# prstrive/SuRF

Hardware: AMD Instinct MI355X
Metric: rays/sec (576x800, 5-view, 128 samp/ray render, whole job) (higher is better)
Workload: dtype f32 (operands split exactly into 3 bf16 pieces, fp32 accumulate)

## Files before the change

### surf_amd/csrc/blend_split.hip

```cpp
#include <math.h>
#include <string.h>

#include "blend_raw.h"
#include "common.h"

namespace {

using namespace blend_raw;

constexpr int TILE = 32;
#ifndef SURF_BLEND_WPB
#define SURF_BLEND_WPB 8
#endif
constexpr int WPB = SURF_BLEND_WPB;

enum { L_RD0, L_RD2, L_B0S, L_B0V, L_B2, L_V0, L_V2, L_W0, L_R0, L_R2, N_L };
constexpr int NKS[N_L] = {1, 1, 3, 2, 4, 2, 2, 2, 3, 1};
constexpr int NT[N_L] = {1, 1, 2, 2, 1, 1, 1, 1, 1, 1};
constexpr int blk_off(int l) { int o = 0; for (int i = 0; i < l; ++i) o += NKS[i] * NT[i]; return o; }
constexpr int N_BLK = blk_off(N_L);
enum { B_RD0, B_RD2, B_B0_T0, B_B0_T1, B_B2, B_V0, B_V2, B_W0, B_R0, B_R2, N_BIAS };
enum { D_VIS, D_VIS2, D_RGB4, N_DOT };
template <int BB> constexpr int bias_off() { return N_BLK * BB; }
template <int BB> constexpr int dot_off() { return bias_off<BB>() + N_BIAS * 128; }
template <int BB> constexpr int scal_off() { return dot_off<BB>() + N_DOT * 128; }
template <int BB> constexpr int image_bytes() { return scal_off<BB>() + 16; }

constexpr float LOG2E = 1.44269504088896341f, LN2 = 0.69314718055994531f;

typedef __bf16 bf16x8 __attribute__((ext_vector_type(8)));
typedef __bf16 bf16x2 __attribute__((ext_vector_type(2)));
typedef _Float16 f16x8 __attribute__((ext_vector_type(8)));
typedef _Float16 f16x2 __attribute__((ext_vector_type(2)));
typedef float f32x2 __attribute__((ext_vector_type(2)));
typedef uint32_t u32x4 __attribute__((ext_vector_type(4)));

template <int NP>
struct FragT { u32x4 p[NP]; };

#ifndef SURF_BLEND_MRES
#define SURF_BLEND_MRES 1
#endif

#ifndef SURF_BLEND_MRES_MASK
#define SURF_BLEND_MRES_MASK 0x3ff
#endif
struct BPolBf3 {
  static constexpr int NP = 3, ID = 1, BB = NP * 1024, LANE_BYTES = 16;
  static constexpr bool MRES = SURF_BLEND_MRES != 0;
  static constexpr bool mres_at(int site) { return MRES && ((SURF_BLEND_MRES_MASK >> site) & 1); }
#ifndef SURF_BLEND_REG_VIEWS_BF3
#define SURF_BLEND_REG_VIEWS_BF3 2
#endif
// ... 331 lines not shown
#endif
}

template <class P> constexpr int lds_bytes() { return image_bytes<P::BB>(); }

constexpr int SLOT_GROUPS = 5;
constexpr int slot_floats(int ns) { return ns * SLOT_GROUPS * 64 * 4; }
#ifndef SURF_BLEND_LDS_VIEWS
#define SURF_BLEND_LDS_VIEWS 2
#endif
constexpr int VIEW_BYTES = SLOT_GROUPS * 64 * 16;
template <class P> constexpr int lds_views() {
  const int n = (160 * 1024 - lds_bytes<P>()) / (WPB * VIEW_BYTES);
  return n < SURF_BLEND_LDS_VIEWS ? n : SURF_BLEND_LDS_VIEWS;
}
struct Stage {
  float* slot;
  char* lds_v;
  int n_lds;
};

struct ViewState {
  float floc[12];
  float rd[4];
  float rgb[3];
  float ex;
  float mk;
};
template <class PtrT>
__device__ __forceinline__ void slot_store_at(PtrT p, const ViewState& s, int stride = 64) {
  p[0 * stride] = f32x4{s.floc[0], s.floc[1], s.floc[2], s.floc[3]};
  p[1 * stride] = f32x4{s.floc[4], s.floc[5], s.floc[6], s.floc[7]};
  p[2 * stride] = f32x4{s.floc[8], s.floc[9], s.floc[10], s.floc[11]};
  p[3 * stride] = f32x4{s.rd[0], s.rd[1], s.rd[2], s.rd[3]};
  p[4 * stride] = f32x4{s.rgb[0], s.rgb[1], s.rgb[2], s.mk != 0.f ? s.ex : -s.ex};
}
template <class PtrT>
__device__ __forceinline__ void slot_load_at(PtrT p, ViewState& s, int stride = 64) {
  f32x4 x[5];
#pragma unroll
  for (int g = 0; g < 5; ++g) x[g] = p[g * stride];
#pragma unroll
  for (int g = 0; g < 3; ++g) {
    s.floc[4 * g + 0] = x[g][0]; s.floc[4 * g + 1] = x[g][1]; s.floc[4 * g + 2] = x[g][2]; s.floc[4 * g + 3] = x[g][3];
  }
  s.rd[0] = x[3][0]; s.rd[1] = x[3][1]; s.rd[2] = x[3][2]; s.rd[3] = x[3][3];
  s.rgb[0] = x[4][0]; s.rgb[1] = x[4][1]; s.rgb[2] = x[4][2];
  s.mk = x[4][3] > 0.f ? 1.f : 0.f;
  s.ex = fabsf(x[4][3]);
}
typedef __attribute__((address_space(3))) f32x4* lds_f32x4_ptr;
struct ViewRegs { f32x4 x[5]; };
template <int NRV> struct RegViews { ViewRegs v0, v1, v2; };
template <int NRV>
__device__ __forceinline__ void slot_store(const Stage& g, int v, int lane, const ViewState& s, RegViews<NRV>& keep) {
  if (v < g.n_lds) { slot_store_at((lds_f32x4_ptr)(g.lds_v + v * VIEW_BYTES), s); return; }
  if (NRV > 0 && v == g.n_lds) { slot_store_at(&keep.v0.x[0], s, 1); return; }
  if (NRV > 1 && v == g.n_lds + 1) { slot_store_at(&keep.v1.x[0], s, 1); return; }
  if (NRV > 2 && v == g.n_lds + 2) { slot_store_at(&keep.v2.x[0], s, 1); return; }
  slot_store_at(reinterpret_cast<f32x4*>(g.slot + (int64_t)(v * SLOT_GROUPS) * 256 + lane * 4), s);
}
template <int NRV>
__device__ __forceinline__ void slot_load(const Stage& g, int v, int lane, ViewState& s, const RegViews<NRV>& keep) {
  if (v < g.n_lds) { slot_load_at((lds_f32x4_ptr)(g.lds_v + v * VIEW_BYTES), s); return; }
  if (NRV > 0 && v == g.n_lds) { slot_load_at(&keep.v0.x[0], s, 1); return; }
  if (NRV > 1 && v == g.n_lds + 1) { slot_load_at(&keep.v1.x[0], s, 1); return; }
  if (NRV > 2 && v == g.n_lds + 2) { slot_load_at(&keep.v2.x[0], s, 1); return; }
  slot_load_at(reinterpret_cast<const f32x4*>(g.slot + (int64_t)(v * SLOT_GROUPS) * 256 + lane * 4), s);
}

struct Geo {
  const float* mapA;
  const float* mapB;
  const float* mapC;
  int HA, WA, HB, WB;
  float scA, scB, cWA, cHA, cWB, cHB, rWA, rHA, rWB, rHB;
  int h;
};
__device__ __forceinline__ Geo make_geo(const BlendArgs& a, int h) {
  Geo g;
  g.h = h;
  g.mapA = h ? a.feats[2] : a.feats[0];
  g.mapB = h ? a.feats[3] : a.feats[1];
  g.mapC = h ? a.feats[2] : a.imgs;
  g.HA = h ? a.hw[4] : a.hw[0]; g.WA = h ? a.hw[5] : a.hw[1];
  g.HB = h ? a.hw[6] : a.hw[2]; g.WB = h ? a.hw[7] : a.hw[3];
  g.scA = h ? 0.25f : 1.0f; g.scB = h ? 0.125f : 0.5f;
  g.cWA = (float)(g.WA - 1) / 2.0f; g.cHA = (float)(g.HA - 1) / 2.0f; g.cWB = (float)(g.WB - 1) / 2.0f; g.cHB = (float)(g.HB - 1) / 2.0f;
  g.rWA = 1.0f / g.cWA; g.rHA = 1.0f / g.cHA; g.rWB = 1.0f / g.cWB; g.rHB = 1.0f / g.cHB;
  return g;
}
struct Fetch {
  Tap4 qA, qB, qC;
  TapGeom gA, gB;
  bool ok;
};
__device__ __forceinline__ void pass1_issue(const BlendArgs& a, const Geo& geo, int cam, float px, float py, float pz, float ax, float ay,
                                        float az, ViewState& st, Fetch& q) {
  const int h = geo.h;
  const float* __restrict__ mapA = geo.mapA;
  const float* __restrict__ mapB = geo.mapB;
  const int HA = geo.HA, WA = geo.WA, HB = geo.HB, WB = geo.WB;
  const float scA = geo.scA, scB = geo.scB, cWA = geo.cWA, cHA = geo.cHA, cWB = geo.cWB, cHB = geo.cHB;
  const float rWA = geo.rWA, rHA = geo.rHA, rWB = geo.rWB, rHB = geo.rHB;
  Tap4& qA = q.qA; Tap4& qB = q.qB; Tap4& qC = q.qC;
  TapGeom& gA = q.gA; TapGeom& gB = q.gB;
  (void)h;
  float bx = a.cpos[cam][0] - px, by = a.cpos[cam][1] - py, bz = a.cpos[cam][2] - pz;
  {
    const float nn = sqrtf(bx * bx + by * by + bz * bz) + 1e-6f;
    bx /= nn; by /= nn; bz /= nn;
  }
  const float ddx = ax - bx, ddy = ay - by, ddz = az - bz;
#ifdef SURF_BX_EXACT_RD
  {
    const float dn = fmaxf(sqrtf(ddx * ddx + ddy * ddy + ddz * ddz), 1e-6f);
    st.rd[0] = ddx / dn; st.rd[1] = ddy / dn; st.rd[2] = ddz / dn;
  }
#else
  {
    const float inv = __builtin_amdgcn_rcpf(fmaxf(__builtin_amdgcn_sqrtf(ddx * ddx + ddy * ddy + ddz * ddz), 1e-6f));
    st.rd[0] = ddx * inv; st.rd[1] = ddy * inv; st.rd[2] = ddz * inv;
  }
#endif
  st.rd[3] = ax * bx + ay * by + az * bz;
  const float* M = a.w2c[cam];
  const float X = M[0] * px + M[1] * py + M[2] * pz + M[3];
  const float Y = M[4] * px + M[5] * py + M[6] * pz + M[7];
  const float Z = M[8] * px + M[9] * py + M[10] * pz + M[11];
  const float* K = a.K[cam];
  const float qx = K[0] * X + K[1] * Y + K[2] * Z;
  const float qy = K[3] * X + K[4] * Y + K[5] * Z;
  const float qz = K[6] * X + K[7] * Y + K[8] * Z;
  const float u0 = qx / qz, v0 = qy / qz;
  bool ok = qz > 0.f;
  {
    const float u = u0 * scA, vv = v0 * scA;
    ok = ok && (u >= 0.f) && (u < (float)WA) && (vv >= 0.f) && (vv < (float)HA);
    const float nx = div_const(u, cWA, rWA) - 1.0f, ny = div_const(vv, cHA, rHA) - 1.0f;
    const float gx = ((nx + 1.0f) * (float)WA - 1.0f) * 0.5f, gy = ((ny + 1.0f) * (float)HA - 1.0f) * 0.5f;
    gA = tap_geom(HA, WA, gx, gy);
    tap_issue(qA, mapA + (int64_t)cam * HA * WA * 4, gA);
    tap_issue(qC, geo.mapC + (int64_t)cam * HA * WA * 4, gA);
  }
  {
    const float u = u0 * scB, vv = v0 * scB;
    ok = ok && (u >= 0.f) && (u < (float)WB) && (vv >= 0.f) && (vv < (float)HB);
    const float nx = div_const(u, cWB, rWB) - 1.0f, ny = div_const(vv, cHB, rHB) - 1.0f;
    const float gx = ((nx + 1.0f) * (float)WB - 1.0f) * 0.5f, gy = ((ny + 1.0f) * (float)HB - 1.0f) * 0.5f;
    gB = tap_geom(HB, WB, gx, gy);
    tap_issue(qB, mapB + (int64_t)cam * HB * WB * 4, gB);
  }
  q.ok = ok;
}
template <class P>
__device__ __forceinline__ bool pass1_finish(const Ctx& c, const Geo& geo, float s_abs, ViewState& st, const Fetch& q) {
  typedef typename P::Frag Frag;
  const int h = geo.h;
  const Tap4& qA = q.qA; const Tap4& qB = q.qB; const Tap4& qC = q.qC;
  const TapGeom& gA = q.gA; const TapGeom& gB = q.gB;
  bool ok = q.ok;
  float d12[12];
  {
    const float bin[2] = {h ? st.rd[1] : st.rd[0], h ? st.rd[3] : st.rd[2]};
    Frag fb, f8;
    frags_from<P, 2, 1>(bin, &fb);
    f32x16 acc1 = bias_row<P>(c, B_RD0);
    mma_layer<P, L_RD0, 0, 1>(c, acc1, &fb);
    elu_make_frags<P, 8, 0>(c, acc1, &f8);
    f32x16 acc2 = bias_row<P>(c, B_RD2);
    mma_layer<P, L_RD2, 0, 1>(c, acc2, &f8);
    elu_rows<12>(acc2, d12);
  }
  const f32x4 tA = tap_finish(qA, gA), tB = tap_finish(qB, gB);
  f32x4 tC = tap_finish(qC, gA);
  if (h != 0) tC = f32x4{0.f, 0.f, 0.f, 0.f};
  ok = ok && (__shfl_xor((int)ok, 32) != 0);
  st.mk = ok ? 1.f : 0.f;
  st.rgb[0] = tC[0]; st.rgb[1] = tC[1]; st.rgb[2] = tC[2];
  float g[12];
  if (h == 0) {
    g[0] = tC[0]; g[1] = tC[1]; g[2] = tC[2];
    g[3] = tA[0]; g[4] = tA[1]; g[5] = tA[2]; g[6] = tA[3];
    g[7] = tB[0]; g[8] = tB[1]; g[9] = tB[2]; g[10] = tB[3];
  } else {
    g[0] = tA[0]; g[1] = tA[1]; g[2] = tA[2]; g[3] = tA[3];
    g[4] = tB[0]; g[5] = tB[1]; g[6] = tB[2]; g[7] = tB[3];
    g[8] = g[9] = g[10] = 0.f;
  }
#pragma unroll
  for (int r = 0; r < 11; ++r) st.floc[r] = g[r] + d12[r];
  st.floc[11] = 0.f;
  st.ex = expf(s_abs * (st.rd[3] - 1.0f));
  return ok;
}

template <class P>
__global__ __launch_bounds__(WPB * 64, WPB / 4) void blend_split_kernel(BlendArgs a) {
  typedef typename P::Frag Frag;
  __shared__ __attribute__((aligned(16))) char lds[lds_bytes<P>() + WPB * lds_views<P>() * VIEW_BYTES];
  static_assert(lds_bytes<P>() % 16 == 0 && lds_bytes<P>() + WPB * lds_views<P>() * VIEW_BYTES <= 160 * 1024, "LDS");
  for (int o = threadIdx.x * 16; o < lds_bytes<P>(); o += WPB * 64 * 16)
    *reinterpret_cast<u32x4*>(lds + o) = *reinterpret_cast<const u32x4*>(a.w + o);
  __syncthreads();

  Ctx c0;
  const int lane = threadIdx.x & 63;
  const int j = lane & 31, h = lane >> 5;
  c0.lds = lds;
  c0.lane16 = lane * 16;
  c0.h64 = h * 64;
  c0.I0 = ident_frag(lane, 0);
  c0.I1 = ident_frag(lane, 1);
  const int NS = a.nv - 1;
  const int64_t wave_id = (int64_t)blockIdx.x * WPB + (threadIdx.x >> 6);
  const int64_t n_waves = (int64_t)gridDim.x * WPB;
  const int64_t n_pts = a.n_dev ? (int64_t)*a.n_dev : a.n;
  const int64_t n_tiles = (n_pts + TILE - 1) / TILE;
  Stage slot;
  slot.slot = a.scratch + wave_id * slot_floats(NS);
  slot.lds_v = lds + lds_bytes<P>() + (threadIdx.x >> 6) * (lds_views<P>() * VIEW_BYTES) + lane * 16;
  slot.n_lds = lds_views<P>();
  const float* scal = reinterpret_cast<const float*>(lds + scal_off<P::BB>());
  const float s_abs = scal[0], b_vis = scal[1], b_vis2 = scal[2], b_rgb4 = scal[3];

  const Geo geo = make_geo(a, h);

#ifdef SURF_BLEND_TIMING
  unsigned long long tprev = __builtin_readcyclecounter(), tacc[8] = {0, 0, 0, 0, 0, 0, 0, 0};
  const unsigned long long t_begin = tprev, rt_begin = __builtin_amdgcn_s_memrealtime();
#endif
  for (int64_t tile = wave_id; tile < n_tiles; tile += n_waves) {
    SURF_BT(0);
    const int64_t slot_i = tile * TILE + j;
    const int64_t sc = slot_i < n_pts ? slot_i : n_pts - 1;
    const int64_t i = a.idx ? (int64_t)a.idx[sc] : sc;
    const bool active = (slot_i < n_pts) && (!a.mask || a.mask[i] != 0);
    if (__ballot(active) == 0ull) continue;
    const float px = a.pts[i * 3 + 0], py = a.pts[i * 3 + 1], pz = a.pts[i * 3 + 2];

    float ax = a.cpos[0][0] - px, ay = a.cpos[0][1] - py, az = a.cpos[0][2] - pz;
    {
      const float nn = sqrtf(ax * ax + ay * ay + az * az) + 1e-6f;
      ax /= nn; ay /= nn; az /= nn;
    }
    int nvalid = 0;
    float emin = INFINITY;
    RegViews<P::REG_VIEWS> keep;
#pragma unroll 1
    for (int v = 0; v < NS; ++v) {
      const Ctx c = opaque(c0);
      ViewState st;
      Fetch q;
      pass1_issue(a, geo, v + 1, px, py, pz, ax, ay, az, st, q);
      nvalid += pass1_finish<P>(c, geo, s_abs, st, q) ? 1 : 0;
      emin = fminf(emin, st.ex);
      slot_store(slot, v, lane, st, keep);
    }
    if (a.n_valid && active && h == 0) a.n_valid[i] = (uint8_t)nvalid;
    SURF_BT(1);

    float wsum = 0.f;
    float mv[24];
#pragma unroll
    for (int ch = 0; ch < 24; ++ch) mv[ch] = 0.f;
#pragma unroll 1
    for (int v = 0; v < NS; ++v) {
      ViewState st;
      slot_load(slot, v, lane, st, keep);
      const float w = (st.ex - emin) * st.mk;
      wsum += w;
#pragma unroll
      for (int ch = 0; ch < 12; ++ch) mv[ch] += st.floc[ch] * w;
    }
    const float winv = 1.0f / (wsum + 1e-8f);
#pragma unroll
    for (int ch = 0; ch < 12; ++ch) mv[ch] *= winv;
#pragma unroll 1
    for (int v = 0; v < NS; ++v) {
      ViewState st;
      slot_load(slot, v, lane, st, keep);
      const float w = (st.ex - emin) * st.mk * winv;
#pragma unroll
      for (int ch = 0; ch < 12; ++ch) { const float d = st.floc[ch] - mv[ch]; mv[12 + ch] += w * (d * d); }
    }
    SURF_BT(2);
    f32x16 G0a, G0b;
    {
      const Ctx c = opaque(c0);
      G0a = bias_row<P>(c, B_B0_T0);
      G0b = bias_row<P>(c, B_B0_T1);
      Frag fm[3];
      make_frags<P, 24, 3, 1>(c, mv, fm);
      mma_layer<P, L_B0S, 0, 3>(c, G0a, fm);
      mma_layer<P, L_B0S, 1, 3>(c, G0b, fm);
    }

    float Mx = -INFINITY, Zs = 0.f, o_r = 0.f, o_g = 0.f, o_b = 0.f;
    SURF_BT(3);
#pragma unroll 1
    for (int v = 0; v < NS; ++v) {
      const Ctx c = opaque(c0);
      ViewState st;
      slot_load(slot, v, lane, st, keep);
      const float wv = (st.ex - emin) * st.mk * winv;
      f32x16 a0 = G0a, a1 = G0b;
      {
        Frag fl[2];
        make_frags<P, 12, 2, 2>(c, st.floc, fl);
        mma_layer<P, L_B0V, 0, 2>(c, a0, fl);
        mma_layer<P, L_B0V, 1, 2>(c, a1, fl);
      }
      f32x16 ax2 = bias_row<P>(c, B_B2);
      {
        Frag hf[2];
        elu_make_frags<P, 16, 3>(c, a0, hf);
        mma_blk<P, L_B2, 0, 0>(c, ax2, hf[0]);
        mma_blk<P, L_B2, 1, 0>(c, ax2, hf[1]);
        SURF_PHASE();
        elu_make_frags<P, 16, 4>(c, a1, hf);
        mma_blk<P, L_B2, 2, 0>(c, ax2, hf[0]);
        mma_blk<P, L_B2, 3, 0>(c, ax2, hf[1]);
        SURF_PHASE();
      }
      float x[16];
      elu_rows<16>(ax2, x);
      SURF_BT(4);
      float vis;
      {
        f32x16 at;
#pragma unroll
        for (int r = 0; r < 16; ++r) at[r] = 0.f;
        {
          Frag xf[2];
          make_frags<P, 16, 2, 5>(c, x, xf);
          mma_layer<P, L_V0, 0, 2>(c, at, xf);
        }
        const f32x16 bt = bias_row<P>(c, B_V0);
        f32x16 ar = bias_row<P>(c, B_V2);
        float vraw = 0.f;
        {
          float t16[16];
#pragma unroll
          for (int r = 0; r < 16; ++r) t16[r] = elu_t(fmaf(at[r], wv, bt[r]));
          const f32x16 dvis = dot_row<P>(c, D_VIS);
#pragma unroll
          for (int r = 0; r < 16; ++r) vraw = fmaf(dvis[r], t16[r], vraw);
          Frag tf[2];
          make_frags<P, 16, 2, 6>(c, t16, tf);
          mma_layer<P, L_V2, 0, 2>(c, ar, tf);
        }
        vraw += __shfl_xor(vraw, 32);
        vis = sigm(elu_x(vraw + b_vis)) * st.mk;
#pragma unroll
        for (int r = 0; r < 16; ++r) x[r] += elu_t(ar[r]);
      }
      SURF_BT(5);
      Frag rf[3];
      make_frags<P, 16, 2, 7>(c, x, rf);
      float vis2;
      {
        f32x16 aw;
#pragma unroll
        for (int r = 0; r < 16; ++r) aw[r] = 0.f;
        mma_layer<P, L_W0, 0, 2>(c, aw, rf);
        const f32x16 bw = bias_row<P>(c, B_W0);
        const f32x16 dvis2 = dot_row<P>(c, D_VIS2);
        float v2 = 0.f;
#pragma unroll
        for (int r = 0; r < 16; ++r) v2 = fmaf(dvis2[r], elu_t(fmaf(aw[r], vis, bw[r])), v2);
        v2 += __shfl_xor(v2, 32);
        vis2 = sigm(v2 + b_vis2) * st.mk;
      }
      SURF_BT(6);
      float rr;
      {
        f32x16 a16 = bias_row<P>(c, B_R0);
        {
          const float extra[3] = {h ? st.rd[0] : vis2, h ? st.rd[2] : st.rd[1], h ? 0.f : st.rd[3]};
          make_frags<P, 3, 1, 8>(c, extra, rf + 2);
          mma_layer<P, L_R0, 0, 3>(c, a16, rf);
        }
        f32x16 a8 = bias_row<P>(c, B_R2);
        {
          Frag f8;
          elu_make_frags<P, 8, 9>(c, a16, &f8);
          mma_layer<P, L_R2, 0, 1>(c, a8, &f8);
        }
        const f32x16 drgb4 = dot_row<P>(c, D_RGB4);
        rr = 0.f;
#pragma unroll
        for (int r = 0; r < 4; ++r) rr = fmaf(drgb4[r], elu_t(a8[r]), rr);
        rr += __shfl_xor(rr, 32);
        rr += b_rgb4;
      }
      if (st.mk == 0.f) rr = -1e9f;
      const float Mn = fmaxf(Mx, rr);
      const float scl = expf(Mx - Mn);
      const float e = expf(rr - Mn);
      Zs = Zs * scl + e;
      o_r = o_r * scl + e * st.rgb[0];
      o_g = o_g * scl + e * st.rgb[1];
      o_b = o_b * scl + e * st.rgb[2];
      Mx = Mn;
      SURF_BT(7);
    }
    if (active && h == 0) {
      a.color[i * 3 + 0] = o_r / Zs;
      a.color[i * 3 + 1] = o_g / Zs;
      a.color[i * 3 + 2] = o_b / Zs;
    }
  }
#ifdef SURF_BLEND_TIMING
  if (threadIdx.x == 0)
    for (int k = 0; k < 8; ++k) atomicAdd(&g_bphase[k], tacc[k]);
  if (threadIdx.x == 0 && blockIdx.x < 256) {
    g_bwg[blockIdx.x][0] = rt_begin;
    g_bwg[blockIdx.x][1] = __builtin_amdgcn_s_memrealtime();
  }
  if (threadIdx.x == 0 && blockIdx.x == 0) {
    g_bphase[8] = __builtin_readcyclecounter() - t_begin;
    g_bphase[9] = __builtin_amdgcn_s_memrealtime() - rt_begin;
  }
#endif
}

int grid_blocks(int64_t n) {
  const int64_t tiles = (n + TILE - 1) / TILE;
  const int64_t blocks = (tiles + WPB - 1) / WPB;
  return (int)(blocks < 256 ? blocks : 256);
}

inline uint16_t bf16_rne(float f) {
  uint32_t u;
  memcpy(&u, &f, 4);
  if ((u & 0x7fffffffu) > 0x7f800000u) return (uint16_t)((u >> 16) | 0x40);
  u += 0x7fffu + ((u >> 16) & 1u);
  return (uint16_t)(u >> 16);
}
inline float bf16_to_f(uint16_t b) {
  uint32_t u = (uint32_t)b << 16;
  float f;
  memcpy(&f, &u, 4);
  return f;
}
inline uint16_t f16_bits(float v) {
  _Float16 hh = (_Float16)v;
  uint16_t b;
  memcpy(&b, &hh, 2);
  return b;
}
inline float f16_to_f(uint16_t b) {
  _Float16 hh;
  memcpy(&hh, &b, 2);
  return (float)hh;
}
template <class P> void split_host(float v, uint16_t* p);
template <> void split_host<BPolBf3>(float v, uint16_t* p) {
  p[0] = bf16_rne(v);
  float r = v - bf16_to_f(p[0]);
  p[1] = bf16_rne(r);
  r = r - bf16_to_f(p[1]);
  p[2] = bf16_rne(r);
}
template <> void split_host<BPolH2>(float v, uint16_t* p) {
  p[0] = f16_bits(v);
  p[1] = f16_bits(v - f16_to_f(p[0]));
}
template <class P> void put_weight(unsigned char* out, int blk, int lane, int i, float v) {
  uint16_t p[P::NP];
  split_host<P>(v, p);
  for (int pc = 0; pc < P::NP; ++pc) reinterpret_cast<uint16_t*>(out + (int64_t)blk * P::BB + pc * 1024 + lane * 16)[i] = p[pc];
}
template <> void put_weight<BPolF32>(unsigned char* out, int blk, int lane, int i, float v) {
  reinterpret_cast<float*>(out + (int64_t)blk * BPolF32::BB + lane * 32)[i] = v;
}

// ... 29 lines not shown
  float* dots = reinterpret_cast<float*>(out + dot_off<P::BB>());
  float* scal = reinterpret_cast<float*>(out + scal_off<P::BB>());
  auto nat_row = [](int lim) { return [lim](int t, int rho) { const int f = 32 * t + rho; return f < lim ? f : -1; }; };
  auto nat_col = [](int lim) { return [lim](int m, int h) { const int f = hk(m / 16, m % 16, h); return f < lim ? f : -1; }; };
  auto natf = [](int lim) { return [lim](int r, int h) { const int f = hk(0, r, h); return f < lim ? f : -1; }; };
  auto dir_row = [](int t, int rho) { const int hr = (rho >> 2) & 1, r = (rho & 3) | ((rho >> 3) << 2); return loc_ch(r, hr); };

  pack_layer<P>(out, L_RD0, raw + R_RD0_W, 4, nat_row(16), [](int m, int h) { return m < 2 ? 2 * m + h : -1; });
  pack_rows(bias + B_RD0 * 32, raw + R_RD0_B, natf(16), LOG2E);
  pack_layer<P>(out, L_RD2, raw + R_RD2_W, 16, dir_row, nat_col(16));
  pack_rows(bias + B_RD2 * 32, raw + R_RD2_B, [](int r, int h) { return loc_ch(r, h); }, LOG2E);
  pack_layer<P>(out, L_B0S, raw + R_B0_W, 57, nat_row(64), [](int m, int h) {
    const int grp = m / 12, s = m % 12;
    const int ch = (grp < 2 && s < 11) ? loc_ch(s, h) : -1;
    return ch >= 0 ? grp * DF + ch : -1;
  });
  pack_rows(bias + B_B0_T0 * 32, raw + R_B0_B, [](int r, int h) { return hk(0, r, h); }, LOG2E);
  pack_rows(bias + B_B0_T1 * 32, raw + R_B0_B, [](int r, int h) { return hk(1, r, h); }, LOG2E);
  pack_layer<P>(out, L_B0V, raw + R_B0_W, 57, nat_row(64), [](int m, int h) {
    const int ch = m < 11 ? loc_ch(m, h) : -1;
    return ch >= 0 ? 2 * DF + ch : -1;
  });
  pack_layer<P>(out, L_B2, raw + R_B2_W, 64, nat_row(32), nat_col(64));
  pack_rows(bias + B_B2 * 32, raw + R_B2_B, natf(32), LOG2E);
  pack_layer<P>(out, L_V0, raw + R_V0_W, 32, nat_row(32), nat_col(32));
  pack_rows(bias + B_V0 * 32, raw + R_V0_B, natf(32), LOG2E);
  pack_layer<P>(out, L_V2, raw + R_V2_W, 32, nat_row(32), nat_col(32));
  pack_rows(bias + B_V2 * 32, raw + R_V2_B, natf(32), LOG2E);
  pack_rows(dots + D_VIS * 32, raw + R_V2_W + 32 * 32, natf(32), 1.0f);
  pack_layer<P>(out, L_W0, raw + R_W0_W, 32, nat_row(32), nat_col(32));
  pack_rows(bias + B_W0 * 32, raw + R_W0_B, natf(32), LOG2E);
  pack_rows(dots + D_VIS2 * 32, raw + R_W2_W, natf(32), 1.0f);
  pack_layer<P>(out, L_R0, raw + R_R0_W, 37, nat_row(16), [](int m, int h) {
    if (m < 16) return hk(0, m, h);
    if (m == 16) return h ? 33 : 32;
    if (m == 17) return h ? 35 : 34;
    if (m == 18) return h ? -1 : 36;
    return -1;
  });
  pack_rows(bias + B_R0 * 32, raw + R_R0_B, natf(16), LOG2E);
  pack_layer<P>(out, L_R2, raw + R_R2_W, 16, nat_row(8), nat_col(16));
  pack_rows(bias + B_R2 * 32, raw + R_R2_B, natf(8), LOG2E);
  pack_rows(dots + D_RGB4 * 32, raw + R_R4_W, [](int r, int h) { return r < 4 ? 4 * h + r : -1; }, 1.0f);
  scal[0] = fabsf(raw[R_S]);
  scal[1] = raw[R_V2_B + 32];
  scal[2] = raw[R_W2_B];
  scal[3] = raw[R_R4_B];
  return 0;
}

template <class P>
int launch(const BlendArgs& a, hipStream_t st) {
  dim3 grid(grid_blocks(a.n)), block(WPB * 64);
  hipLaunchKernelGGL((blend_split_kernel<P>), grid, block, 0, st, a);
  return surf_check_launch();
}

}

#ifdef SURF_BLEND_TIMING
extern "C" int surf_debug_blend_wg(unsigned long long* out) {
  return hipMemcpyFromSymbol(out, HIP_SYMBOL(g_bwg), sizeof(unsigned long long) * 512) == hipSuccess ? 0 : 100;
}
extern "C" int surf_debug_blend_phases(unsigned long long* out, int reset) {
  if (hipMemcpyFromSymbol(out, HIP_SYMBOL(g_bphase), sizeof(unsigned long long) * 10) != hipSuccess) return 100;
  if (reset) {
    unsigned long long z[10] = {0, 0, 0, 0, 0, 0, 0, 0, 0, 0};
    if (hipMemcpyToSymbol(HIP_SYMBOL(g_bphase), z, sizeof(z)) != hipSuccess) return 100;
  }
  return 0;
}
#endif

extern "C" int64_t surf_blend_split_packed_bytes(int precision) {
  if (precision == BPolBf3::ID) return image_bytes<BPolBf3::BB>();
  if (precision == BPolH2::ID) return image_bytes<BPolH2::BB>();
  if (precision == BPolF32::ID) return image_bytes<BPolF32::BB>();
  return SURF_E_ARG;
}

extern "C" int surf_blend_pack_weights_split(const float* h_raw, unsigned char* h_packed, int precision) {
  if (precision == BPolBf3::ID) return pack_weights<BPolBf3>(h_raw, h_packed);
  if (precision == BPolH2::ID) return pack_weights<BPolH2>(h_raw, h_packed);
  if (precision == BPolF32::ID) return pack_weights<BPolF32>(h_raw, h_packed);
  return SURF_E_ARG;
}

extern "C" int64_t surf_blend_split_scratch_bytes(int64_t n_points, int nv) {
  if (n_points <= 0 || nv < 2 || nv > SURF_MAX_VIEWS) return 0;
  return (int64_t)grid_blocks(n_points) * WPB * slot_floats(nv - 1) * (int64_t)sizeof(float);
}

static int blend_split_impl(const float* pts, const uint8_t* mask, const int32_t* idx, int64_t n, const int32_t* d_n,
                            const float* const* h_feats, const int* h_hw, int n_level, const float* imgs, int nv,
                            const float* h_intrs, const float* h_w2c, const float* h_c2w, const void* blend_w,
                            int precision, float* color, uint8_t* n_valid, void* scratch, void* stream) {
  if (!pts || !h_feats || !h_hw || !imgs || !h_intrs || !h_w2c || !h_c2w || !blend_w || !color || !scratch) return SURF_E_ARG;
  if (n <= 0 || nv < 2) return SURF_E_ARG;
  if (n_level != 4 || nv > SURF_MAX_VIEWS) return SURF_E_LIMIT;
  if (precision != BPolBf3::ID && precision != BPolH2::ID && precision != BPolF32::ID) return SURF_E_ARG;
  BlendArgs a;
  a.pts = pts; a.mask = mask; a.idx = idx; a.n = n; a.n_dev = d_n; a.imgs = imgs; a.w = (const unsigned char*)blend_w; a.color = color;
  a.n_valid = n_valid;
  a.scratch = (float*)scratch;
  a.nv = nv;
  for (int l = 0; l < 4; ++l) {
    if (!h_feats[l]) return SURF_E_ARG;
// ... 35 lines not shown
```

Baseline: 3.010 million.

## Share per-view geometry across wave halves and split register-view paths statically

Each wave half now computes the camera geometry (ray direction, exp weight, projection) for a different view, and the results are exchanged with ds_bpermute, so two views cost one geometry computation per lane. The register-kept views are peeled out of the runtime-indexed loops into static calls, which removes the dynamic branch chain in slot load and store and may help keep those views in registers. The tap selection in pass1_finish becomes per-element selects instead of a divergent branch. The price is extra cross-lane permutes and somewhat more complex control flow.

```diff
diff --git a/surf_amd/csrc/blend_split.hip b/surf_amd/csrc/blend_split.hip
--- a/surf_amd/csrc/blend_split.hip
+++ b/surf_amd/csrc/blend_split.hip
@@ -436,13 +436,24 @@
 typedef __attribute__((address_space(3))) f32x4* lds_f32x4_ptr;
 struct ViewRegs { f32x4 x[5]; };
 template <int NRV> struct RegViews { ViewRegs v0, v1, v2; };
-template <int NRV>
-__device__ __forceinline__ void slot_store(const Stage& g, int v, int lane, const ViewState& s, RegViews<NRV>& keep) {
+__device__ __forceinline__ void slot_store_mem(const Stage& g, int v, int lane, const ViewState& s) {
   if (v < g.n_lds) { slot_store_at((lds_f32x4_ptr)(g.lds_v + v * VIEW_BYTES), s); return; }
-  if (NRV > 0 && v == g.n_lds) { slot_store_at(&keep.v0.x[0], s, 1); return; }
-  if (NRV > 1 && v == g.n_lds + 1) { slot_store_at(&keep.v1.x[0], s, 1); return; }
-  if (NRV > 2 && v == g.n_lds + 2) { slot_store_at(&keep.v2.x[0], s, 1); return; }
   slot_store_at(reinterpret_cast<f32x4*>(g.slot + (int64_t)(v * SLOT_GROUPS) * 256 + lane * 4), s);
+}
+__device__ __forceinline__ void slot_load_mem(const Stage& g, int v, int lane, ViewState& s) {
+  if (v < g.n_lds) { slot_load_at((lds_f32x4_ptr)(g.lds_v + v * VIEW_BYTES), s); return; }
+  slot_load_at(reinterpret_cast<const f32x4*>(g.slot + (int64_t)(v * SLOT_GROUPS) * 256 + lane * 4), s);
+}
+template <int NRV, class KeepT, class MemF, class RegF>
+__device__ __forceinline__ void for_views_in_order(int NS, int n_lds, KeepT& keep, MemF mem, RegF reg) {
+  const int n0 = NS < n_lds ? NS : n_lds;
+#pragma unroll 1
+  for (int v = 0; v < n0; ++v) mem(v);
+  if (NRV > 0 && NS > n_lds) reg(n_lds, keep.v0);
+  if (NRV > 1 && NS > n_lds + 1) reg(n_lds + 1, keep.v1);
+  if (NRV > 2 && NS > n_lds + 2) reg(n_lds + 2, keep.v2);
+#pragma unroll 1
+  for (int v = n_lds + NRV; v < NS; ++v) mem(v);
 }
 template <int NRV>
 __device__ __forceinline__ void slot_load(const Stage& g, int v, int lane, ViewState& s, const RegViews<NRV>& keep) {
@@ -479,8 +490,57 @@
   TapGeom gA, gB;
   bool ok;
 };
-__device__ __forceinline__ void pass1_issue(const BlendArgs& a, const Geo& geo, int cam, float px, float py, float pz, float ax, float ay,
-                                        float az, ViewState& st, Fetch& q) {
+struct P1Geom {
+  float rd[4];
+  float ex, u0, v0;
+  int front;
+};
+__device__ __forceinline__ P1Geom pass1_geom(const BlendArgs& a, int cam, float px, float py, float pz, float ax, float ay, float az,
+                                             float s_abs) {
+  P1Geom g;
+  float bx = a.cpos[cam][0] - px, by = a.cpos[cam][1] - py, bz = a.cpos[cam][2] - pz;
+  {
+    const float nn = sqrtf(bx * bx + by * by + bz * bz) + 1e-6f;
+    bx /= nn; by /= nn; bz /= nn;
+  }
+  const float ddx = ax - bx, ddy = ay - by, ddz = az - bz;
+#ifdef SURF_BX_EXACT_RD
+  {
+    const float dn = fmaxf(sqrtf(ddx * ddx + ddy * ddy + ddz * ddz), 1e-6f);
+    g.rd[0] = ddx / dn; g.rd[1] = ddy / dn; g.rd[2] = ddz / dn;
+  }
+#else
+  {
+    const float inv = __builtin_amdgcn_rcpf(fmaxf(__builtin_amdgcn_sqrtf(ddx * ddx + ddy * ddy + ddz * ddz), 1e-6f));
+    g.rd[0] = ddx * inv; g.rd[1] = ddy * inv; g.rd[2] = ddz * inv;
+  }
+#endif
+  g.rd[3] = ax * bx + ay * by + az * bz;
+  g.ex = expf(s_abs * (g.rd[3] - 1.0f));
+  const float* M = a.w2c[cam];
+  const float X = M[0] * px + M[1] * py + M[2] * pz + M[3];
+  const float Y = M[4] * px + M[5] * py + M[6] * pz + M[7];
+  const float Z = M[8] * px + M[9] * py + M[10] * pz + M[11];
+  const float* K = a.K[cam];
+  const float qx = K[0] * X + K[1] * Y + K[2] * Z;
+  const float qy = K[3] * X + K[4] * Y + K[5] * Z;
+  const float qz = K[6] * X + K[7] * Y + K[8] * Z;
+  g.u0 = qx / qz; g.v0 = qy / qz;
+  g.front = qz > 0.f ? 1 : 0;
+  return g;
+}
+__device__ __forceinline__ P1Geom geom_of_half(const P1Geom& g, int t, int lane) {
+  const int src = (((lane & 31) | (t << 5)) << 2);
+  P1Geom o;
+#pragma unroll
+  for (int k = 0; k < 4; ++k) o.rd[k] = __builtin_bit_cast(float, __builtin_amdgcn_ds_bpermute(src, __builtin_bit_cast(int, g.rd[k])));
+  o.ex = __builtin_bit_cast(float, __builtin_amdgcn_ds_bpermute(src, __builtin_bit_cast(int, g.ex)));
+  o.u0 = __builtin_bit_cast(float, __builtin_amdgcn_ds_bpermute(src, __builtin_bit_cast(int, g.u0)));
+  o.v0 = __builtin_bit_cast(float, __builtin_amdgcn_ds_bpermute(src, __builtin_bit_cast(int, g.v0)));
+  o.front = __builtin_amdgcn_ds_bpermute(src, g.front);
+  return o;
+}
+__device__ __forceinline__ void pass1_issue(const Geo& geo, int cam, const P1Geom& pg, ViewState& st, Fetch& q) {
   const int h = geo.h;
   const float* __restrict__ mapA = geo.mapA;
   const float* __restrict__ mapB = geo.mapB;
@@ -490,34 +550,10 @@
   Tap4& qA = q.qA; Tap4& qB = q.qB; Tap4& qC = q.qC;
   TapGeom& gA = q.gA; TapGeom& gB = q.gB;
   (void)h;
-  float bx = a.cpos[cam][0] - px, by = a.cpos[cam][1] - py, bz = a.cpos[cam][2] - pz;
-  {
-    const float nn = sqrtf(bx * bx + by * by + bz * bz) + 1e-6f;
-    bx /= nn; by /= nn; bz /= nn;
-  }
-  const float ddx = ax - bx, ddy = ay - by, ddz = az - bz;
-#ifdef SURF_BX_EXACT_RD
-  {
-    const float dn = fmaxf(sqrtf(ddx * ddx + ddy * ddy + ddz * ddz), 1e-6f);
-    st.rd[0] = ddx / dn; st.rd[1] = ddy / dn; st.rd[2] = ddz / dn;
-  }
-#else
-  {
-    const float inv = __builtin_amdgcn_rcpf(fmaxf(__builtin_amdgcn_sqrtf(ddx * ddx + ddy * ddy + ddz * ddz), 1e-6f));
-    st.rd[0] = ddx * inv; st.rd[1] = ddy * inv; st.rd[2] = ddz * inv;
-  }
-#endif
-  st.rd[3] = ax * bx + ay * by + az * bz;
-  const float* M = a.w2c[cam];
-  const float X = M[0] * px + M[1] * py + M[2] * pz + M[3];
-  const float Y = M[4] * px + M[5] * py + M[6] * pz + M[7];
-  const float Z = M[8] * px + M[9] * py + M[10] * pz + M[11];
-  const float* K = a.K[cam];
-  const float qx = K[0] * X + K[1] * Y + K[2] * Z;
-  const float qy = K[3] * X + K[4] * Y + K[5] * Z;
-  const float qz = K[6] * X + K[7] * Y + K[8] * Z;
-  const float u0 = qx / qz, v0 = qy / qz;
-  bool ok = qz > 0.f;
+  st.rd[0] = pg.rd[0]; st.rd[1] = pg.rd[1]; st.rd[2] = pg.rd[2]; st.rd[3] = pg.rd[3];
+  st.ex = pg.ex;
+  const float u0 = pg.u0, v0 = pg.v0;
+  bool ok = pg.front != 0;
   {
     const float u = u0 * scA, vv = v0 * scA;
     ok = ok && (u >= 0.f) && (u < (float)WA) && (vv >= 0.f) && (vv < (float)HA);
@@ -538,7 +574,7 @@
   q.ok = ok;
 }
 template <class P>
-__device__ __forceinline__ bool pass1_finish(const Ctx& c, const Geo& geo, float s_abs, ViewState& st, const Fetch& q) {
+__device__ __forceinline__ bool pass1_finish(const Ctx& c, const Geo& geo, ViewState& st, const Fetch& q) {
   typedef typename P::Frag Frag;
   const int h = geo.h;
   const Tap4& qA = q.qA; const Tap4& qB = q.qB; const Tap4& qC = q.qC;
@@ -562,20 +598,16 @@
   ok = ok && (__shfl_xor((int)ok, 32) != 0);
   st.mk = ok ? 1.f : 0.f;
   st.rgb[0] = tC[0]; st.rgb[1] = tC[1]; st.rgb[2] = tC[2];
+  const bool h0 = h == 0;
   float g[12];
-  if (h == 0) {
-    g[0] = tC[0]; g[1] = tC[1]; g[2] = tC[2];
-    g[3] = tA[0]; g[4] = tA[1]; g[5] = tA[2]; g[6] = tA[3];
-    g[7] = tB[0]; g[8] = tB[1]; g[9] = tB[2]; g[10] = tB[3];
-  } else {
-    g[0] = tA[0]; g[1] = tA[1]; g[2] = tA[2]; g[3] = tA[3];
-    g[4] = tB[0]; g[5] = tB[1]; g[6] = tB[2]; g[7] = tB[3];
-    g[8] = g[9] = g[10] = 0.f;
-  }
+  g[0] = h0 ? tC[0] : tA[0]; g[1] = h0 ? tC[1] : tA[1]; g[2] = h0 ? tC[2] : tA[2];
+  g[3] = h0 ? tA[0] : tA[3];
+  g[4] = h0 ? tA[1] : tB[0]; g[5] = h0 ? tA[2] : tB[1]; g[6] = h0 ? tA[3] : tB[2];
+  g[7] = h0 ? tB[0] : tB[3];
+  g[8] = h0 ? tB[1] : 0.f; g[9] = h0 ? tB[2] : 0.f; g[10] = h0 ? tB[3] : 0.f;
 #pragma unroll
   for (int r = 0; r < 11; ++r) st.floc[r] = g[r] + d12[r];
   st.floc[11] = 0.f;
-  st.ex = expf(s_abs * (st.rd[3] - 1.0f));
   return ok;
 }
 
@@ -631,15 +663,40 @@
     int nvalid = 0;
     float emin = INFINITY;
     RegViews<P::REG_VIEWS> keep;
+    auto pass1_geom_pair = [&](int vA, int vB) { return pass1_geom(a, (h ? vB : vA) + 1, px, py, pz, ax, ay, az, s_abs); };
+    auto pass1_view = [&](int v, const P1Geom& pair, int t, ViewState& st) {
+      const Ctx c = opaque(c0);
+      Fetch q;
+      pass1_issue(geo, v + 1, geom_of_half(pair, t, lane), st, q);
+      nvalid += pass1_finish<P>(c, geo, st, q) ? 1 : 0;
+      emin = fminf(emin, st.ex);
+    };
+    auto pass1_single = [&](int v, ViewState& st) {
+      const Ctx c = opaque(c0);
+      Fetch q;
+      pass1_issue(geo, v + 1, pass1_geom(a, v + 1, px, py, pz, ax, ay, az, s_abs), st, q);
+      nvalid += pass1_finish<P>(c, geo, st, q) ? 1 : 0;
+      emin = fminf(emin, st.ex);
+    };
+    {
+      constexpr int NRV = P::REG_VIEWS;
+      const int n_lds = slot.n_lds;
+      const int k = NS <= n_lds ? NS : (NS > n_lds + NRV ? NS - NRV : n_lds);
+      auto m = [&](int i) { return i < n_lds ? i : i + NRV; };
 #pragma unroll 1
-    for (int v = 0; v < NS; ++v) {
-      const Ctx c = opaque(c0);
-      ViewState st;
-      Fetch q;
-      pass1_issue(a, geo, v + 1, px, py, pz, ax, ay, az, st, q);
-      nvalid += pass1_finish<P>(c, geo, s_abs, st, q) ? 1 : 0;
-      emin = fminf(emin, st.ex);
-      slot_store(slot, v, lane, st, keep);
+      for (int i = 0; i < k; i += 2) {
+        const int cnt = k - i < 2 ? k - i : 2;
+        const P1Geom pair = pass1_geom_pair(m(i), m(i + cnt - 1));
+#pragma unroll 1
+        for (int t = 0; t < cnt; ++t) {
+          ViewState st;
+          pass1_view(m(i + t), pair, t, st);
+          slot_store_mem(slot, m(i + t), lane, st);
+        }
+      }
+      if (NRV > 0 && NS > n_lds) { ViewState st; pass1_single(n_lds, st); slot_store_at(&keep.v0.x[0], st, 1); }
+      if (NRV > 1 && NS > n_lds + 1) { ViewState st; pass1_single(n_lds + 1, st); slot_store_at(&keep.v1.x[0], st, 1); }
+      if (NRV > 2 && NS > n_lds + 2) { ViewState st; pass1_single(n_lds + 2, st); slot_store_at(&keep.v2.x[0], st, 1); }
     }
     if (a.n_valid && active && h == 0) a.n_valid[i] = (uint8_t)nvalid;
     SURF_BT(1);
@@ -648,26 +705,28 @@
     float mv[24];
 #pragma unroll
     for (int ch = 0; ch < 24; ++ch) mv[ch] = 0.f;
-#pragma unroll 1
-    for (int v = 0; v < NS; ++v) {
-      ViewState st;
-      slot_load(slot, v, lane, st, keep);
+    auto mean_view = [&](const ViewState& st) {
       const float w = (st.ex - emin) * st.mk;
       wsum += w;
 #pragma unroll
       for (int ch = 0; ch < 12; ++ch) mv[ch] += st.floc[ch] * w;
-    }
+    };
+    for_views_in_order<P::REG_VIEWS>(
+        NS, slot.n_lds, keep,
+        [&](int v) { ViewState st; slot_load_mem(slot, v, lane, st); mean_view(st); },
+        [&](int, const ViewRegs& r) { ViewState st; slot_load_at(&r.x[0], st, 1); mean_view(st); });
     const float winv = 1.0f / (wsum + 1e-8f);
 #pragma unroll
     for (int ch = 0; ch < 12; ++ch) mv[ch] *= winv;
-#pragma unroll 1
-    for (int v = 0; v < NS; ++v) {
-      ViewState st;
-      slot_load(slot, v, lane, st, keep);
+    auto var_view = [&](const ViewState& st) {
       const float w = (st.ex - emin) * st.mk * winv;
 #pragma unroll
       for (int ch = 0; ch < 12; ++ch) { const float d = st.floc[ch] - mv[ch]; mv[12 + ch] += w * (d * d); }
-    }
+    };
+    for_views_in_order<P::REG_VIEWS>(
+        NS, slot.n_lds, keep,
+        [&](int v) { ViewState st; slot_load_mem(slot, v, lane, st); var_view(st); },
+        [&](int, const ViewRegs& r) { ViewState st; slot_load_at(&r.x[0], st, 1); var_view(st); });
     SURF_BT(2);
     f32x16 G0a, G0b;
     {
```

New measurement: 3.025 million, median of 4. About the same (+0.5%).

## Skip blend MLP for wave-uniformly masked views; add optional cross-tile fetch lookahead

Applied to the files above, without the earlier changes.

Pass 2 of the blend kernel now skips the whole per-view MLP chain (B0/B2/V/W/R layers) when no lane in the wave has a valid mask for that view, and sets the logit to -1e9 directly. This is on by default for multi-piece precision forms. The kernel is also split into a templated body, and a software-pipelined pass 1 that issues the next tile's and next view's texture taps ahead of the current MLP work is added. That pipelining is disabled by default behind SURF_BLEND_LOOKAHEAD, and an env var can select the old form. The skip adds a ballot per view and more divergence in control flow, while lookahead would raise register pressure.

```diff
diff --git a/surf_amd/csrc/blend_split.hip b/surf_amd/csrc/blend_split.hip
--- a/surf_amd/csrc/blend_split.hip
+++ b/surf_amd/csrc/blend_split.hip
@@ -1,4 +1,5 @@
 #include <math.h>
+#include <stdlib.h>
 #include <string.h>
 
 #include "blend_raw.h"
@@ -478,7 +479,9 @@
   Tap4 qA, qB, qC;
   TapGeom gA, gB;
   bool ok;
-};
+  unsigned long long okm;
+};
+template <bool AHEAD = false>
 __device__ __forceinline__ void pass1_issue(const BlendArgs& a, const Geo& geo, int cam, float px, float py, float pz, float ax, float ay,
                                         float az, ViewState& st, Fetch& q) {
   const int h = geo.h;
@@ -525,7 +528,7 @@
     const float gx = ((nx + 1.0f) * (float)WA - 1.0f) * 0.5f, gy = ((ny + 1.0f) * (float)HA - 1.0f) * 0.5f;
     gA = tap_geom(HA, WA, gx, gy);
     tap_issue(qA, mapA + (int64_t)cam * HA * WA * 4, gA);
-    tap_issue(qC, geo.mapC + (int64_t)cam * HA * WA * 4, gA);
+    if (!AHEAD) tap_issue(qC, geo.mapC + (int64_t)cam * HA * WA * 4, gA);
   }
   {
     const float u = u0 * scB, vv = v0 * scB;
@@ -535,16 +538,16 @@
     gB = tap_geom(HB, WB, gx, gy);
     tap_issue(qB, mapB + (int64_t)cam * HB * WB * 4, gB);
   }
-  q.ok = ok;
+  if (AHEAD) q.okm = __ballot(ok);
+  else q.ok = ok;
+}
+__device__ __forceinline__ void pass1_issue_c(const Geo& geo, int cam, Fetch& q) {
+  tap_issue(q.qC, geo.mapC + (int64_t)cam * geo.HA * geo.WA * 4, q.gA);
 }
 template <class P>
-__device__ __forceinline__ bool pass1_finish(const Ctx& c, const Geo& geo, float s_abs, ViewState& st, const Fetch& q) {
+__device__ __forceinline__ void pass1_dir(const Ctx& c, const Geo& geo, const ViewState& st, float (&d12)[12]) {
   typedef typename P::Frag Frag;
   const int h = geo.h;
-  const Tap4& qA = q.qA; const Tap4& qB = q.qB; const Tap4& qC = q.qC;
-  const TapGeom& gA = q.gA; const TapGeom& gB = q.gB;
-  bool ok = q.ok;
-  float d12[12];
   {
     const float bin[2] = {h ? st.rd[1] : st.rd[0], h ? st.rd[3] : st.rd[2]};
     Frag fb, f8;
@@ -556,6 +559,13 @@
     mma_layer<P, L_RD2, 0, 1>(c, acc2, &f8);
     elu_rows<12>(acc2, d12);
   }
+}
+template <class P, bool AHEAD = false>
+__device__ __forceinline__ bool pass1_taps(const Geo& geo, float s_abs, ViewState& st, const Fetch& q, const float (&d12)[12]) {
+  const int h = geo.h;
+  const Tap4& qA = q.qA; const Tap4& qB = q.qB; const Tap4& qC = q.qC;
+  const TapGeom& gA = q.gA; const TapGeom& gB = q.gB;
+  bool ok = AHEAD ? ((q.okm >> (threadIdx.x & 63)) & 1ull) != 0 : q.ok;
   const f32x4 tA = tap_finish(qA, gA), tB = tap_finish(qB, gB);
   f32x4 tC = tap_finish(qC, gA);
   if (h != 0) tC = f32x4{0.f, 0.f, 0.f, 0.f};
@@ -578,12 +588,46 @@
   st.ex = expf(s_abs * (st.rd[3] - 1.0f));
   return ok;
 }
-
 template <class P>
-__global__ __launch_bounds__(WPB * 64, WPB / 4) void blend_split_kernel(BlendArgs a) {
+__device__ __forceinline__ bool pass1_finish(const Ctx& c, const Geo& geo, float s_abs, ViewState& st, const Fetch& q) {
+  float d12[12];
+  pass1_dir<P>(c, geo, st, d12);
+  return pass1_taps<P>(geo, s_abs, st, q, d12);
+}
+
+struct TilePt {
+  int64_t i;
+  bool active;
+  float px, py, pz, ax, ay, az;
+};
+__device__ __forceinline__ TilePt load_point(const BlendArgs& a, int64_t tile, int j, int64_t n_pts) {
+  TilePt p;
+  const int64_t slot_i = tile * TILE + j;
+  const int64_t sc = slot_i < n_pts ? slot_i : n_pts - 1;
+  p.i = a.idx ? (int64_t)a.idx[sc] : sc;
+  p.active = (slot_i < n_pts) && (!a.mask || a.mask[p.i] != 0);
+  p.px = a.pts[p.i * 3 + 0]; p.py = a.pts[p.i * 3 + 1]; p.pz = a.pts[p.i * 3 + 2];
+  return p;
+}
+__device__ __forceinline__ void ref_dir(const BlendArgs& a, TilePt& p) {
+  p.ax = a.cpos[0][0] - p.px; p.ay = a.cpos[0][1] - p.py; p.az = a.cpos[0][2] - p.pz;
+  const float nn = sqrtf(p.ax * p.ax + p.ay * p.ay + p.az * p.az) + 1e-6f;
+  p.ax /= nn; p.ay /= nn; p.az /= nn;
+}
+
+#ifndef SURF_BLEND_SKIP
+#define SURF_BLEND_SKIP 1
+#endif
+#ifndef SURF_BLEND_LA_ORDER
+#define SURF_BLEND_LA_ORDER 1
+#endif
+#ifndef SURF_BLEND_LOOKAHEAD
+#define SURF_BLEND_LOOKAHEAD 0
+#endif
+template <class P, int FORM>
+__device__ __forceinline__ void blend_split_body(const BlendArgs& a, char* lds) {
   typedef typename P::Frag Frag;
-  __shared__ __attribute__((aligned(16))) char lds[lds_bytes<P>() + WPB * lds_views<P>() * VIEW_BYTES];
-  static_assert(lds_bytes<P>() % 16 == 0 && lds_bytes<P>() + WPB * lds_views<P>() * VIEW_BYTES <= 160 * 1024, "LDS");
+  constexpr bool SKIP = FORM != 0 && SURF_BLEND_SKIP != 0, LA = FORM != 0 && SURF_BLEND_LOOKAHEAD != 0;
   for (int o = threadIdx.x * 16; o < lds_bytes<P>(); o += WPB * 64 * 16)
     *reinterpret_cast<u32x4*>(lds + o) = *reinterpret_cast<const u32x4*>(a.w + o);
   __syncthreads();
@@ -614,32 +658,87 @@
   unsigned long long tprev = __builtin_readcyclecounter(), tacc[8] = {0, 0, 0, 0, 0, 0, 0, 0};
   const unsigned long long t_begin = tprev, rt_begin = __builtin_amdgcn_s_memrealtime();
 #endif
+  TilePt pt;
+  Fetch fa, fb;
+  ViewState sa, sb;
+  if constexpr (LA) {
+    if (wave_id < n_tiles) {
+      pt = load_point(a, wave_id, j, n_pts);
+      ref_dir(a, pt);
+      pass1_issue<true>(a, geo, 1, pt.px, pt.py, pt.pz, pt.ax, pt.ay, pt.az, sa, fa);
+    }
+  }
   for (int64_t tile = wave_id; tile < n_tiles; tile += n_waves) {
     SURF_BT(0);
-    const int64_t slot_i = tile * TILE + j;
-    const int64_t sc = slot_i < n_pts ? slot_i : n_pts - 1;
-    const int64_t i = a.idx ? (int64_t)a.idx[sc] : sc;
-    const bool active = (slot_i < n_pts) && (!a.mask || a.mask[i] != 0);
-    if (__ballot(active) == 0ull) continue;
-    const float px = a.pts[i * 3 + 0], py = a.pts[i * 3 + 1], pz = a.pts[i * 3 + 2];
-
-    float ax = a.cpos[0][0] - px, ay = a.cpos[0][1] - py, az = a.cpos[0][2] - pz;
-    {
-      const float nn = sqrtf(ax * ax + ay * ay + az * az) + 1e-6f;
-      ax /= nn; ay /= nn; az /= nn;
+    TilePt p, pnx;
+    if constexpr (LA) {
+      p = pt;
+      ref_dir(a, p);
+      const int64_t tnext = tile + n_waves < n_tiles ? tile + n_waves : tile;
+      pnx = load_point(a, tnext, j, n_pts);
+      pt = pnx;
+      if (__ballot(p.active) == 0ull) {
+        ref_dir(a, pnx);
+        pass1_issue<true>(a, geo, 1, pnx.px, pnx.py, pnx.pz, pnx.ax, pnx.ay, pnx.az, sa, fa);
+        continue;
+      }
+    } else {
+      const int64_t slot_i = tile * TILE + j;
+      const int64_t sc = slot_i < n_pts ? slot_i : n_pts - 1;
+      p.i = a.idx ? (int64_t)a.idx[sc] : sc;
+      p.active = (slot_i < n_pts) && (!a.mask || a.mask[p.i] != 0);
+      if (__ballot(p.active) == 0ull) continue;
+      p.px = a.pts[p.i * 3 + 0]; p.py = a.pts[p.i * 3 + 1]; p.pz = a.pts[p.i * 3 + 2];
+      ref_dir(a, p);
     }
+    const int64_t i = p.i;
+    const bool active = p.active;
+    const float px = p.px, py = p.py, pz = p.pz, ax = p.ax, ay = p.ay, az = p.az;
     int nvalid = 0;
     float emin = INFINITY;
     RegViews<P::REG_VIEWS> keep;
+    if constexpr (LA) {
+      ref_dir(a, pnx);
+      auto issue = [&](bool next_tile, int cam, ViewState& s, Fetch& q) {
+        pass1_issue<true>(a, geo, next_tile ? 1 : cam, next_tile ? pnx.px : px, next_tile ? pnx.py : py, next_tile ? pnx.pz : pz,
+                           next_tile ? pnx.ax : ax, next_tile ? pnx.ay : ay, next_tile ? pnx.az : az, s, q);
+      };
+      auto step = [&](int v, ViewState& s, Fetch& q, bool next_tile, int cam_next, ViewState& sn, Fetch& qn) {
+        if (SURF_BLEND_LA_ORDER == 0) issue(next_tile, cam_next, sn, qn);
+        pass1_issue_c(geo, v + 1, q);
+        SURF_PHASE();
+        const Ctx c = opaque(c0);
+        float d12[12];
+        pass1_dir<P>(c, geo, s, d12);
+        if (SURF_BLEND_LA_ORDER != 0) {
+          issue(next_tile, cam_next, sn, qn);
+          SURF_PHASE();
+        }
+        nvalid += pass1_taps<P, true>(geo, s_abs, s, q, d12) ? 1 : 0;
+        emin = fminf(emin, s.ex);
+        slot_store(slot, v, lane, s, keep);
+      };
 #pragma unroll 1
-    for (int v = 0; v < NS; ++v) {
-      const Ctx c = opaque(c0);
-      ViewState st;
-      Fetch q;
-      pass1_issue(a, geo, v + 1, px, py, pz, ax, ay, az, st, q);
-      nvalid += pass1_finish<P>(c, geo, s_abs, st, q) ? 1 : 0;
-      emin = fminf(emin, st.ex);
-      slot_store(slot, v, lane, st, keep);
+      for (int v = 0; v < NS; v += 2) {
+        step(v, sa, fa, v + 1 >= NS, v + 2, sb, fb);
+        if (v + 1 >= NS) {
+          fa = fb;
+          sa.rd[0] = sb.rd[0]; sa.rd[1] = sb.rd[1]; sa.rd[2] = sb.rd[2]; sa.rd[3] = sb.rd[3];
+          break;
+        }
+        step(v + 1, sb, fb, v + 2 >= NS, v + 3, sa, fa);
+      }
+    } else {
+#pragma unroll 1
+      for (int v = 0; v < NS; ++v) {
+        const Ctx c = opaque(c0);
+        ViewState st;
+        Fetch q;
+        pass1_issue(a, geo, v + 1, px, py, pz, ax, ay, az, st, q);
+        nvalid += pass1_finish<P>(c, geo, s_abs, st, q) ? 1 : 0;
+        emin = fminf(emin, st.ex);
+        slot_store(slot, v, lane, st, keep);
+      }
     }
     if (a.n_valid && active && h == 0) a.n_valid[i] = (uint8_t)nvalid;
     SURF_BT(1);
@@ -687,98 +786,100 @@
       const Ctx c = opaque(c0);
       ViewState st;
       slot_load(slot, v, lane, st, keep);
-      const float wv = (st.ex - emin) * st.mk * winv;
-      f32x16 a0 = G0a, a1 = G0b;
-      {
-        Frag fl[2];
-        make_frags<P, 12, 2, 2>(c, st.floc, fl);
-        mma_layer<P, L_B0V, 0, 2>(c, a0, fl);
-        mma_layer<P, L_B0V, 1, 2>(c, a1, fl);
+      float rr = -1e9f;
+      if (!(SKIP && __ballot(st.mk != 0.f) == 0ull)) {
+        const float wv = (st.ex - emin) * st.mk * winv;
+        f32x16 a0 = G0a, a1 = G0b;
+        {
+          Frag fl[2];
+          make_frags<P, 12, 2, 2>(c, st.floc, fl);
+          mma_layer<P, L_B0V, 0, 2>(c, a0, fl);
+          mma_layer<P, L_B0V, 1, 2>(c, a1, fl);
+        }
+        f32x16 ax2 = bias_row<P>(c, B_B2);
+        {
+          Frag hf[2];
+          elu_make_frags<P, 16, 3>(c, a0, hf);
+          mma_blk<P, L_B2, 0, 0>(c, ax2, hf[0]);
+          mma_blk<P, L_B2, 1, 0>(c, ax2, hf[1]);
+          SURF_PHASE();
+          elu_make_frags<P, 16, 4>(c, a1, hf);
+          mma_blk<P, L_B2, 2, 0>(c, ax2, hf[0]);
+          mma_blk<P, L_B2, 3, 0>(c, ax2, hf[1]);
+          SURF_PHASE();
+        }
+        float x[16];
+        elu_rows<16>(ax2, x);
+        SURF_BT(4);
+        float vis;
+        {
+          f32x16 at;
+#pragma unroll
+          for (int r = 0; r < 16; ++r) at[r] = 0.f;
+          {
+            Frag xf[2];
+            make_frags<P, 16, 2, 5>(c, x, xf);
+            mma_layer<P, L_V0, 0, 2>(c, at, xf);
+          }
+          const f32x16 bt = bias_row<P>(c, B_V0);
+          f32x16 ar = bias_row<P>(c, B_V2);
+          float vraw = 0.f;
+          {
+            float t16[16];
+#pragma unroll
+            for (int r = 0; r < 16; ++r) t16[r] = elu_t(fmaf(at[r], wv, bt[r]));
+            const f32x16 dvis = dot_row<P>(c, D_VIS);
+#pragma unroll
+            for (int r = 0; r < 16; ++r) vraw = fmaf(dvis[r], t16[r], vraw);
+            Frag tf[2];
+            make_frags<P, 16, 2, 6>(c, t16, tf);
+            mma_layer<P, L_V2, 0, 2>(c, ar, tf);
+          }
+          vraw += __shfl_xor(vraw, 32);
+          vis = sigm(elu_x(vraw + b_vis)) * st.mk;
+#pragma unroll
+          for (int r = 0; r < 16; ++r) x[r] += elu_t(ar[r]);
+        }
+        SURF_BT(5);
+        Frag rf[3];
+        make_frags<P, 16, 2, 7>(c, x, rf);
+        float vis2;
+        {
+          f32x16 aw;
+#pragma unroll
+          for (int r = 0; r < 16; ++r) aw[r] = 0.f;
+          mma_layer<P, L_W0, 0, 2>(c, aw, rf);
+          const f32x16 bw = bias_row<P>(c, B_W0);
+          const f32x16 dvis2 = dot_row<P>(c, D_VIS2);
+          float v2 = 0.f;
+#pragma unroll
+          for (int r = 0; r < 16; ++r) v2 = fmaf(dvis2[r], elu_t(fmaf(aw[r], vis, bw[r])), v2);
+          v2 += __shfl_xor(v2, 32);
+          vis2 = sigm(v2 + b_vis2) * st.mk;
+        }
+        SURF_BT(6);
+        {
+          f32x16 a16 = bias_row<P>(c, B_R0);
+          {
+            const float extra[3] = {h ? st.rd[0] : vis2, h ? st.rd[2] : st.rd[1], h ? 0.f : st.rd[3]};
+            make_frags<P, 3, 1, 8>(c, extra, rf + 2);
+            mma_layer<P, L_R0, 0, 3>(c, a16, rf);
+          }
+          f32x16 a8 = bias_row<P>(c, B_R2);
+          {
+            Frag f8;
+            elu_make_frags<P, 8, 9>(c, a16, &f8);
+            mma_layer<P, L_R2, 0, 1>(c, a8, &f8);
+          }
+          const f32x16 drgb4 = dot_row<P>(c, D_RGB4);
+          rr = 0.f;
+#pragma unroll
+          for (int r = 0; r < 4; ++r) rr = fmaf(drgb4[r], elu_t(a8[r]), rr);
+          rr += __shfl_xor(rr, 32);
+          rr += b_rgb4;
+        }
+        if (st.mk == 0.f) rr = -1e9f;
       }
-      f32x16 ax2 = bias_row<P>(c, B_B2);
-      {
-        Frag hf[2];
-        elu_make_frags<P, 16, 3>(c, a0, hf);
-        mma_blk<P, L_B2, 0, 0>(c, ax2, hf[0]);
-        mma_blk<P, L_B2, 1, 0>(c, ax2, hf[1]);
-        SURF_PHASE();
-        elu_make_frags<P, 16, 4>(c, a1, hf);
-        mma_blk<P, L_B2, 2, 0>(c, ax2, hf[0]);
-        mma_blk<P, L_B2, 3, 0>(c, ax2, hf[1]);
-        SURF_PHASE();
-      }
-      float x[16];
-      elu_rows<16>(ax2, x);
-      SURF_BT(4);
-      float vis;
-      {
-        f32x16 at;
-#pragma unroll
-        for (int r = 0; r < 16; ++r) at[r] = 0.f;
-        {
-          Frag xf[2];
-          make_frags<P, 16, 2, 5>(c, x, xf);
-          mma_layer<P, L_V0, 0, 2>(c, at, xf);
-        }
-        const f32x16 bt = bias_row<P>(c, B_V0);
-        f32x16 ar = bias_row<P>(c, B_V2);
-        float vraw = 0.f;
-        {
-          float t16[16];
-#pragma unroll
-          for (int r = 0; r < 16; ++r) t16[r] = elu_t(fmaf(at[r], wv, bt[r]));
-          const f32x16 dvis = dot_row<P>(c, D_VIS);
-#pragma unroll
-          for (int r = 0; r < 16; ++r) vraw = fmaf(dvis[r], t16[r], vraw);
-          Frag tf[2];
-          make_frags<P, 16, 2, 6>(c, t16, tf);
-          mma_layer<P, L_V2, 0, 2>(c, ar, tf);
-        }
-        vraw += __shfl_xor(vraw, 32);
-        vis = sigm(elu_x(vraw + b_vis)) * st.mk;
-#pragma unroll
-        for (int r = 0; r < 16; ++r) x[r] += elu_t(ar[r]);
-      }
-      SURF_BT(5);
-      Frag rf[3];
-      make_frags<P, 16, 2, 7>(c, x, rf);
-      float vis2;
-      {
-        f32x16 aw;
-#pragma unroll
-        for (int r = 0; r < 16; ++r) aw[r] = 0.f;
-        mma_layer<P, L_W0, 0, 2>(c, aw, rf);
-        const f32x16 bw = bias_row<P>(c, B_W0);
-        const f32x16 dvis2 = dot_row<P>(c, D_VIS2);
-        float v2 = 0.f;
-#pragma unroll
-        for (int r = 0; r < 16; ++r) v2 = fmaf(dvis2[r], elu_t(fmaf(aw[r], vis, bw[r])), v2);
-        v2 += __shfl_xor(v2, 32);
-        vis2 = sigm(v2 + b_vis2) * st.mk;
-      }
-      SURF_BT(6);
-      float rr;
-      {
-        f32x16 a16 = bias_row<P>(c, B_R0);
-        {
-          const float extra[3] = {h ? st.rd[0] : vis2, h ? st.rd[2] : st.rd[1], h ? 0.f : st.rd[3]};
-          make_frags<P, 3, 1, 8>(c, extra, rf + 2);
-          mma_layer<P, L_R0, 0, 3>(c, a16, rf);
-        }
-        f32x16 a8 = bias_row<P>(c, B_R2);
-        {
-          Frag f8;
-          elu_make_frags<P, 8, 9>(c, a16, &f8);
-          mma_layer<P, L_R2, 0, 1>(c, a8, &f8);
-        }
-        const f32x16 drgb4 = dot_row<P>(c, D_RGB4);
-        rr = 0.f;
-#pragma unroll
-        for (int r = 0; r < 4; ++r) rr = fmaf(drgb4[r], elu_t(a8[r]), rr);
-        rr += __shfl_xor(rr, 32);
-        rr += b_rgb4;
-      }
-      if (st.mk == 0.f) rr = -1e9f;
       const float Mn = fmaxf(Mx, rr);
       const float scl = expf(Mx - Mn);
       const float e = expf(rr - Mn);
@@ -807,6 +908,19 @@
     g_bphase[9] = __builtin_amdgcn_s_memrealtime() - rt_begin;
   }
 #endif
+}
+
+template <class P> constexpr int lds_total() { return lds_bytes<P>() + WPB * lds_views<P>() * VIEW_BYTES; }
+template <class P>
+__global__ __launch_bounds__(WPB * 64, WPB / 4) void blend_split_kernel(BlendArgs a) {
+  __shared__ __attribute__((aligned(16))) char lds[lds_total<P>()];
+  static_assert(lds_bytes<P>() % 16 == 0 && lds_total<P>() <= 160 * 1024, "LDS");
+  blend_split_body<P, P::NP == 1 ? 0 : 1>(a, lds);
+}
+template <class P>
+__global__ __launch_bounds__(WPB * 64, WPB / 4) void blend_split_kernel_form0(BlendArgs a) {
+  __shared__ __attribute__((aligned(16))) char lds[lds_total<P>()];
+  blend_split_body<P, 0>(a, lds);
 }
 
 int grid_blocks(int64_t n) {
@@ -942,7 +1056,11 @@
 template <class P>
 int launch(const BlendArgs& a, hipStream_t st) {
   dim3 grid(grid_blocks(a.n)), block(WPB * 64);
-  hipLaunchKernelGGL((blend_split_kernel<P>), grid, block, 0, st, a);
+  const char* form_env = getenv("SURF_BLEND_FORM");
+  if (form_env && form_env[0] == '0' && form_env[1] == 0)
+    hipLaunchKernelGGL((blend_split_kernel_form0<P>), grid, block, 0, st, a);
+  else
+    hipLaunchKernelGGL((blend_split_kernel<P>), grid, block, 0, st, a);
   return surf_check_launch();
 }
 
```

Result: no change. 3.105 million before, 3.115 million after, median of 4 (+0.3%).
